# Blaizzy/mlx-audio

Hardware: AMD Instinct MI355X
Metric: audio samples/sec + real-time factor, Kokoro-82M TTS (higher is better)
Workload: dtype bf16 weights x fp32 activations: vocoder convs = fp16 hi pass (v_mfma_f32_32x32x16_f16) + block-scaled FP4 (e2m1) lo pass (v_mfma_scale_f32_32x32x64_f8f6f4 cbsz / blgp 4, OCP MX: E8M0 scale per row x 32 channels / per output column), fp32 accumulate; front end bf16 hi+lo split; 1 GPU; Kokoro-82M bf16 TTS, tokens->waveform, canonical short sentence T=80 F=264 (6.6 s @ 24 kHz); utterances_per_gpu=64, global_batch=64, samples_per_utterance=158400, parallelism=utterance-dp1, precision_mode=6, wire=fp32

## Files before the change

include/mi355audio.h:

```cpp
#ifndef MI355AUDIO_H
#define MI355AUDIO_H

#include <stdint.h>

#ifdef __cplusplus
extern "C" {
#endif

#define MI355_OK 0
#define MI355_ERR_ARG (-1)
#define MI355_ERR_LAUNCH (-2)
#define MI355_ERR_UNSUPPORTED (-3)

const char* mi355_last_error(void);
int mi355_abi_version(void);
int mi355_device_info(int dev, char* name, int name_cap, int* cu_count, int* lds_bytes);

enum { MI355_ACT_NONE = 0, MI355_ACT_LEAKY = 1, MI355_ACT_SNAKE = 2, MI355_ACT_GELU = 3,
       MI355_ACT_ELU = 4,
       MI355_ACT_SILU = 5,
       MI355_ACT_GELU_TANH = 6,
       MI355_ACT_TANH = 7 };

typedef struct {
// ... 334 lines not shown
  float* y; int64_t y_rstride;
} mi355_interp1d_args;
int mi355_interpolate1d(const mi355_interp1d_args* a, void* stream);

int mi355_conv1d_c1_k3s2(const float* x, int32_t ldx_b, int32_t Lin, const int32_t* lens_in,
                         float w0, float w1, float w2, float bias, float* y, int64_t y_bstride, int32_t ldy, int32_t col,
                         int32_t Lout, int32_t B, void* stream);

typedef struct {
  const float* f0; int32_t ld_f0; int32_t L2; const int32_t* lens2; int32_t B;
  int32_t up; int32_t H; float sr; float sine_amp; float noise_std; float voiced_thr;
  const float* rand_ini; const float* noise;
  const float* lin_w; float lin_b;
  float* phase_ws;
  float* out; int32_t ld_out;
  float* quant_ws;
  int32_t coarse_f32;
} mi355_sine_source_args;
int mi355_sine_source(const mi355_sine_source_args* a, void* stream);

typedef struct {
  const float* x; int32_t ldx; int32_t L; const int32_t* lens; int32_t B;
  int32_t n_fft; int32_t hop; const float* window;
  float* y; int64_t y_bstride; int32_t ldy;
} mi355_stft_magphase_args;
int mi355_stft_magphase(const mi355_stft_magphase_args* a, void* stream);

typedef struct {
  const float* x; int64_t x_bstride; int32_t ldx; int32_t Fr; const int32_t* lens; int32_t B;
  int32_t n_fft; int32_t hop; const float* window;
  float* audio; int32_t ld_audio;
} mi355_istft_head_args;
int mi355_istft_head(const mi355_istft_head_args* a, void* stream);

typedef struct {
  const float* x; int64_t x_bstride; int32_t ldx; int32_t Cin; int32_t L; const int32_t* lens; int32_t B;
  const uint16_t* w; const float* bias; int32_t Cout; int32_t K; int32_t dil; int32_t pad;
  int32_t pre_act; float pre_slope; int32_t precision;
  int32_t n_fft; int32_t hop; const float* window;
  float* audio; int32_t ld_audio;
} mi355_conv_post_istft_args;
int mi355_conv_post_istft(const mi355_conv_post_istft_args* a, void* stream);

typedef struct {
  const float* x; int64_t x_bstride; int32_t ldx; int32_t Cin; int32_t L; const int32_t* lens; int32_t B;
  const uint16_t* w; const float* bias; int32_t Cout; int32_t K; int32_t u; int32_t p; int32_t row_off;
  float slope; int32_t precision;
  const float* res; int64_t res_bstride; int32_t ldr;
  float* y; int64_t y_bstride; int32_t ldy;
} mi355_upsample_polyphase_args;
int mi355_upsample_polyphase(const mi355_upsample_polyphase_args* a, void* stream);

typedef struct {
  const float* x; int32_t ldx; int32_t L; int32_t B;
  int32_t n_fft; int32_t hop; const float* window;
  int32_t pad_mode; int32_t n_frames;
  float* out;
} mi355_stft_args;
int mi355_stft(const mi355_stft_args* a, void* stream);

typedef struct {
  const float* x; int32_t ldx; int32_t L; int32_t B;
  int32_t n_fft; int32_t hop; const float* window; int32_t pad_mode; int32_t n_frames;
  const float* fb; int32_t n_mels; int32_t mode;
  float* out;
  float* gmax;
  float log_guard;
} mi355_logmel_args;
int mi355_logmel(const mi355_logmel_args* a, void* stream);
int mi355_logmel_finish(float* y, int64_t n_per_item, const float* gmax, int32_t B, void* stream);

typedef struct {
  const float* x; int32_t L;
  int32_t win; int32_t shift; int32_t pad; int32_t n_fft; int32_t n_frames;
  const float* window;
  const float* noise;
  float dither; float preemph;
  float* frames;
} mi355_kaldi_frames_args;
int mi355_kaldi_frames(const mi355_kaldi_frames_args* a, void* stream);
int mi355_polar_spec(const float* x, int64_t x_bstride, int32_t ldx, int32_t Fr, int32_t nb, int32_t B, float clip, float* spec, void* stream);


typedef struct {
  const float* spec; int32_t n_frames; int32_t B;
  int32_t n_fft; int32_t hop; const float* window; const float* norm;
  int32_t norm_mode;
  int32_t clamp; int32_t trim; int32_t out_len;
  float* frames_ws;
  float* out; int32_t ld_out;
} mi355_istft_args;
int mi355_istft(const mi355_istft_args* a, void* stream);

enum { MI355_KV_F32 = 0, MI355_KV_BF16 = 1, MI355_KV_F16 = 2 };
typedef struct {
  const float* q; int64_t q_bstride; int32_t ldq;
  const float* k; int64_t k_bstride; int32_t ldk;
  const float* v; int64_t v_bstride; int32_t ldv;
  int32_t heads; int32_t kv_heads; int32_t dh;
  int32_t Tq; int32_t Tk;
  const int32_t* lens_q;
  const int32_t* lens_k;
  int32_t causal; int32_t window; float scale;
  int32_t B;
  int32_t mode;
  float* out; int64_t out_bstride; int32_t ldo;
// ... 443 lines not shown
```

mlx_audio_amd/build.py:

```python
from __future__ import annotations

import hashlib
import os
import shutil
import subprocess
import sys

HERE = os.path.dirname(os.path.abspath(__file__))
CSRC = os.path.join(HERE, "csrc")
LIBDIR = os.path.join(HERE, "lib")
LIBPATH = os.path.join(LIBDIR, "libmi355audio.so")
HEADER = os.path.join(os.path.dirname(HERE), "include", "mi355audio.h")
SOURCES = ["api.cpp", "conv_gemm.hip", "conv_ws4.hip", "conv_ws4_p4.hip", "conv_ws4_p13.hip", "conv_ws4_p5.hip", "conv_ws4_p6.hip", "conv_ws4_p5_probe.hip", "conv_ws4_fq.hip", "upsample_poly.hip", "conv_quant.hip", "norm.hip", "group_norm.hip", "s3.hip", "conformer.hip", "narrow_attn.hip", "mid_attn.hip", "align.hip", "lstm.hip", "lstm_seq.hip", "gru.hip", "dfn.hip", "bandsplit.hip", "sanm.hip", "mossformer.hip", "attention.hip", "glue.hip", "source.hip", "fft.hip", "flash_attn.hip",
           "decode_rules.hip", "gemv.hip", "gemv_mfma.hip", "gemv_mfma_fp8.hip", "gemm_rows.hip", "rows_pipe.hip", "transformer.hip", "rvq.hip", "ecapa.hip", "sampler.hip", "stack_step.cpp", "firered.hip"]
EXTRA_FLAGS = {"source.hip": ["-ffp-contract=off"], "dfn.hip": ["-ffp-contract=off"]}
COMMON_FLAGS = ["-fno-slp-vectorize"]


def _hipcc() -> str:
    for cand in (os.environ.get("HIPCC"), shutil.which("hipcc"), "/opt/rocm/bin/hipcc"):
        if cand and os.path.exists(cand):
            return cand
    raise RuntimeError("hipcc not found (set HIPCC=/path/to/hipcc)")


def _fingerprint() -> str:
    h = hashlib.sha256()
    for name in SOURCES + sorted(n for n in os.listdir(CSRC) if n.endswith(".h")):
        with open(os.path.join(CSRC, name), "rb") as f:
            h.update(f.read())
    with open(HEADER, "rb") as f:
        h.update(f.read())
    h.update(repr(sorted(EXTRA_FLAGS.items())).encode())
    h.update(repr(COMMON_FLAGS).encode())
    return h.hexdigest()


def build(force: bool = False, verbose: bool = True) -> str:
    os.makedirs(LIBDIR, exist_ok=True)
    stamp = os.path.join(LIBDIR, "libmi355audio.stamp")
    fp = _fingerprint()
    if not force and os.path.exists(LIBPATH) and os.path.exists(stamp) and open(stamp).read().strip() == fp:
        return LIBPATH
    hipcc = _hipcc()
    objs = []
    objdir = os.path.join(LIBDIR, "obj")
    os.makedirs(objdir, exist_ok=True)
    procs = []
    for src in SOURCES:
        obj = os.path.join(objdir, src.rsplit(".", 1)[0] + ".o")
        objs.append(obj)
        cmd = [hipcc, "--offload-arch=gfx950", "-O3", "-std=c++17", "-fPIC", *COMMON_FLAGS, *EXTRA_FLAGS.get(src, []), "-x", "hip", "-c",
               os.path.join(CSRC, src), "-o", obj]
        if verbose:
            print("[build]", " ".join(cmd), flush=True)
        procs.append((src, subprocess.Popen(cmd, stdout=subprocess.PIPE, stderr=subprocess.STDOUT, text=True)))
    for src, p in procs:
        out, _ = p.communicate()
        if p.returncode != 0:
            raise RuntimeError(f"hipcc failed on {src}:\n{out}")
        if verbose and out.strip():
            print(out)
    link = [hipcc, "--offload-arch=gfx950", "-shared", "-fPIC", "-o", LIBPATH] + objs
    if verbose:
        print("[build]", " ".join(link), flush=True)
    r = subprocess.run(link, stdout=subprocess.PIPE, stderr=subprocess.STDOUT, text=True)
# ... 10 lines not shown
```

mlx_audio_amd/ops.py:

```python
from __future__ import annotations

import ctypes
import math
import os
from dataclasses import dataclass
from typing import Optional, Tuple

import numpy as np
import torch

from . import _lib

ACT_NONE, ACT_LEAKY, ACT_SNAKE, ACT_GELU, ACT_ELU, ACT_SILU, ACT_GELU_TANH, ACT_TANH = 0, 1, 2, 3, 4, 5, 6, 7

PROFILE = None


def _stream() -> int:
    return torch.cuda.current_stream().cuda_stream


def profile_finalize(entries):
    torch.cuda.synchronize()
    out = []
# ... 1557 lines not shown
            PROFILE.append(((L * B) if lens is None else lens.sum(), pc.cin, pc.cout, pc.k, dil, 0, e0, e1))
        _lib.call_struct("mi355_conv_post_istft", "mi355_conv_post_istft_args", _stream(), x=_ptr(x), x_bstride=xbs, ldx=ldx, Cin=pc.cin, L=L,
                         lens=_ptr(lens), B=B, w=_ptr(pc.w), bias=_ptr(pc.bias), Cout=pc.cout, K=pc.k, dil=dil, pad=pad, pre_act=pre_act,
                         pre_slope=pre_slope, precision=precision, n_fft=n_fft, hop=hop, window=_ptr(window), audio=_ptr(audio),
                         ld_audio=audio.stride(0))
        if PROFILE is not None:
            e1.record()
        return audio
    post = torch.empty((B, L, round_up(pc.cout, 4)), dtype=torch.float32, device=x.device)[:, :, :pc.cout]
    conv_gemm(x, pc, post, dil=dil, pad=pad, lens_in=lens, lens_out=lens, pre_act=pre_act, pre_slope=pre_slope, precision=precision, pre_fq=pre_fq)
    return istft_head(post, n_fft, hop, window, audio, lens=lens)


UPSAMPLE_POLY_SHAPES = {(512, 256, 10): 32, (256, 128, 6): 64}


def upsample_polyphase_eligible(pc: PackedConv, stride: int, *, pre_act: int = ACT_LEAKY, precision: int = 2, res=True, pre_fq=None) -> bool:
    return (pc.k == 2 and stride > 0 and pc.cout % stride == 0 and (pc.cin, pc.cout // stride, stride) in UPSAMPLE_POLY_SHAPES
            and pre_act == ACT_LEAKY and precision == 2 and not pc.f16 and not pc.mx and res is not None and pre_fq is None)


def upsample_polyphase(x: torch.Tensor, pc: PackedConv, res: torch.Tensor, y: torch.Tensor, stride: int, *, row_off: int = 0, lens=None,
                       pre_act: int = ACT_LEAKY, pre_slope: float = 0.1, precision: int = 2, pre_fq=None):
    B, L, _, xbs, ldx = _nlc(x)
    u = stride
    cout = pc.cout // u
    kfull = pc.k * u
    p = (kfull - u) // 2
    Lo = L * u + row_off
    assert y.shape[0] == B and y.shape[1] >= Lo and y.shape[2] == cout and res.shape[0] == B and res.shape[1] >= Lo and res.shape[2] == cout
    if upsample_polyphase_eligible(pc, u, pre_act=pre_act, precision=precision, res=res, pre_fq=pre_fq) and row_off in (0, 1):
        _, _, _, rbs, ldr = _nlc(res)
        _, _, _, ybs, ldy = _nlc(y)
        assert pc.w.numel() >= _lib.load().mi355_packed_conv_weight_elems(pc.cout, pc.k, pc.cin)
        if PROFILE is not None:
            e0, e1 = torch.cuda.Event(enable_timing=True), torch.cuda.Event(enable_timing=True)
            e0.record()
            PROFILE.append((((L + 1) * B) if lens is None else (lens + 1).sum(), pc.cin, pc.cout, pc.k, 1, 1, e0, e1))
        _lib.call_struct("mi355_upsample_polyphase", "mi355_upsample_polyphase_args", _stream(), x=_ptr(x), x_bstride=xbs, ldx=ldx, Cin=pc.cin, L=L,
                         lens=_ptr(lens), B=B, w=_ptr(pc.w), bias=_ptr(pc.bias), Cout=cout, K=kfull, u=u, p=p, row_off=row_off, slope=pre_slope,
                         precision=precision, res=_ptr(res), res_bstride=rbs, ldr=ldr, y=_ptr(y), y_bstride=ybs, ldy=ldy)
        if PROFILE is not None:
            e1.record()
        return y
    kp = pc.k
    conv_gemm(x, pc, y, pad=kp - 1, lout=L + kp - 1, lens_in=lens, lens_out=None if lens is None else lens + (kp - 1), pre_act=pre_act,
              pre_slope=pre_slope, res=res, precision=precision, pre_fq=pre_fq,
              up=dict(s=u, p=p, cout=cout, row_off=row_off, lout=L * u, lens=None if lens is None else lens * u))
    if row_off:
        y[:, :row_off, :].copy_(res[:, :row_off, :])
    return y


def stft_frames(x: torch.Tensor, n_fft: int, hop: int, window: torch.Tensor, pad_mode: int, n_frames: int):
    assert x.dim() == 2 and x.stride(1) == 1 and x.dtype == torch.float32
    B, L = x.shape
    out = torch.empty((B, n_frames, n_fft // 2 + 1, 2), dtype=torch.float32, device=x.device)
    _lib.call_struct("mi355_stft", "mi355_stft_args", _stream(), x=_ptr(x), ldx=x.stride(0), L=L, B=B, n_fft=n_fft, hop=hop,
                     window=_ptr(window), pad_mode=pad_mode, n_frames=n_frames, out=_ptr(out))
    return torch.view_as_complex(out)


def logmel(x: torch.Tensor, n_fft: int, hop: int, window: torch.Tensor, pad_mode: int, n_frames: int, fb: torch.Tensor,
           mode: int, log_guard: float = 0.0, fixed_max: Optional[float] = None):
    assert x.dim() == 2 and x.stride(1) == 1 and fb.is_contiguous()
    B, L = x.shape
    n_mels = fb.shape[0]
    out = torch.empty((B, n_frames, n_mels), dtype=torch.float32, device=x.device)
    gmax = torch.empty((B,), dtype=torch.float32, device=x.device) if mode == 0 else None
    _lib.call_struct("mi355_logmel", "mi355_logmel_args", _stream(), x=_ptr(x), ldx=x.stride(0), L=L, B=B, n_fft=n_fft,
                     hop=hop, window=_ptr(window), pad_mode=pad_mode, n_frames=n_frames, fb=_ptr(fb), n_mels=n_mels,
                     mode=mode, out=_ptr(out), gmax=None if fixed_max is not None else _ptr(gmax), log_guard=float(log_guard))
    if mode == 0:
        if fixed_max is not None:
            gmax.fill_(float(fixed_max))
        lib = _lib.load()
        rc = lib.mi355_logmel_finish(_ptr(out), n_frames * n_mels, _ptr(gmax), B, _stream())
        _lib.check(rc, "mi355_logmel_finish")
    return out


def kaldi_frames(x: torch.Tensor, win: int, shift: int, pad: int, n_fft: int, n_frames: int, window: torch.Tensor, preemph: float,
                 noise: Optional[torch.Tensor] = None, dither: float = 0.0) -> torch.Tensor:
    assert x.dim() == 1 and x.is_contiguous() and x.dtype == torch.float32 and window.numel() == win
    out = torch.empty((n_frames, n_fft), dtype=torch.float32, device=x.device)
    if noise is not None:
        assert noise.is_contiguous() and tuple(noise.shape) == (n_frames, win)
    _lib.call_struct("mi355_kaldi_frames", "mi355_kaldi_frames_args", _stream(), x=_ptr(x), L=x.numel(), win=win, shift=shift, pad=pad, n_fft=n_fft,
                     n_frames=n_frames, window=_ptr(window), noise=_ptr(noise), dither=dither, preemph=preemph, frames=_ptr(out))
    return out


def polar_spec(x: torch.Tensor, nb: int, clip: float = 1e2) -> torch.Tensor:
    B, Fr, C, xbs, ldx = _nlc(x)
    assert C >= 2 * nb
    spec = torch.empty((B, Fr, nb), dtype=torch.complex64, device=x.device)
    lib = _lib.load()
    rc = lib.mi355_polar_spec(_ptr(x), xbs, ldx, Fr, nb, B, float(clip), _ptr(torch.view_as_real(spec)), _stream())
    _lib.check(rc, "mi355_polar_spec")
    return spec


def istft_frames(spec: torch.Tensor, n_fft: int, hop: int, window: torch.Tensor, norm: torch.Tensor, norm_mode: int,
                 clamp: bool, trim: int, out_len: int):
    sr = torch.view_as_real(spec.contiguous())
    B, n_frames = spec.shape[0], spec.shape[1]
# ... 121 lines not shown
```

mlx_audio_amd/tts/models/kokoro/engine.py:

```python
from __future__ import annotations

import math
import os
from dataclasses import dataclass, field
from typing import Dict, List, Optional, Sequence

import numpy as np
import torch

from .... import ops
from ....ops import ACT_GELU, ACT_GELU_TANH, ACT_LEAKY, ACT_NONE, ACT_SNAKE, PackedConv, round_up


def fold_weight_norm(v: torch.Tensor, g: torch.Tensor, param_dtype: torch.dtype) -> torch.Tensor:
    v_ = v.to(param_dtype)
    g_ = g.to(param_dtype)
    axes = tuple(range(1, v_.dim()))
    nrm = torch.sqrt((v_ * v_).sum(dim=axes, keepdim=True))
    w = (v_ / (nrm + torch.tensor(1e-7, dtype=param_dtype))) * g_
    return w.to(torch.float32)


@dataclass
class _AdaIN:
# ... 92 lines not shown
        return torch.cat([hdr, self.ids[i].to(torch.int32).view(torch.float32), self.dur[i].to(torch.int32).view(torch.float32),
                          self.ref_s[i].reshape(-1).to(torch.float32), self.d[i].reshape(-1).to(torch.float32)])

    @staticmethod
    def packed_size(T: int, style: int, width: int) -> int:
        return 1 + 2 * T + style + T * width

    @classmethod
    def unpack(cls, blobs: Sequence[torch.Tensor], frames: Sequence[int], style: int, width: int, speed: float = 1.0) -> "KokoroFront":
        ids, dur, ref, d = [], [], [], []
        for b in blobs:
            T = (int(b.numel()) - 1 - style) // (2 + width)
            ids.append(b[1:1 + T].view(torch.int32))
            dur.append(b[1 + T:1 + 2 * T].view(torch.int32))
            ref.append(b[1 + 2 * T:1 + 2 * T + style])
            d.append(b[1 + 2 * T + style:].reshape(T, width))
        return cls(ids, torch.stack(ref, 0), d, dur, list(frames), speed, None)

    @classmethod
    def concat(cls, parts: Sequence["KokoroFront"]) -> "KokoroFront":
        parts = [p for p in parts if len(p.ids)]
        return cls(sum((p.ids for p in parts), []), torch.cat([p.ref_s for p in parts], 0), sum((p.d for p in parts), []),
                   sum((p.dur for p in parts), []), sum((list(p.frames) for p in parts), []), parts[0].speed, None)


class KokoroEngine:
    ffn_act = ACT_GELU
    alpha_name = "alpha{w}.{i}"
    max_frames = 0
    coarse_f32 = False

    def _decoder_dims(self, config: dict):
        return 1024, 512, 64

    @staticmethod
    def default_precision(param_dtype, quant_modules: Sequence[str] = ()) -> int:
        if param_dtype == torch.float32:
            return 4
        return 6 if (param_dtype == torch.bfloat16 and not tuple(quant_modules)) else 2

    def __init__(self, weights: Dict[str, torch.Tensor], config: dict, device="cuda", param_dtype=torch.bfloat16,
                 precision: Optional[int] = None, quant_modules: Sequence[str] = ()):
        ops.require_gpu()
        self.cfg = config
        self.qmods = tuple(quant_modules)
        if precision is None:
            precision = self.default_precision(param_dtype, self.qmods)
        self.all_f16 = precision == 4
        self.cdim, self.gdim, self.adim = self._decoder_dims(config)
        self.dev = torch.device(device)
        self.pdt = param_dtype
        self.precision = precision
        self.fuse_stats = True
        self.fold_quant = os.environ.get("MI355_FOLD_QUANT", "1") != "0"
        self.ext_partials = os.environ.get("MI355_EXT_PARTIALS", "1") != "0"
        self.w = weights
        ist = config["istftnet"]
        self.rates = [int(r) for r in ist["upsample_rates"]]
        self.kers = [int(k) for k in ist["upsample_kernel_sizes"]]
        self.n_fft, self.hop = int(ist["gen_istft_n_fft"]), int(ist["gen_istft_hop_size"])
        self.total_up = int(np.prod(self.rates)) * self.hop
        self.rk = list(ist["resblock_kernel_sizes"])
        self.rd = [list(d) for d in ist["resblock_dilation_sizes"]]
        self.hid = config["hidden_dim"]
        self.sty = config["style_dim"]
        self.n_layer = config["n_layer"]
        self.pb = config["plbert"]
        self.bank_dec = _StyleBank()
        self.bank_pred = _StyleBank()
        self._load()

    def _t(self, name) -> torch.Tensor:
        return self.w[name].to(torch.float32)

    def _q(self, t: torch.Tensor) -> torch.Tensor:
        return t.to(self.pdt).to(torch.float32)

    def _lin(self, pre, bias=True) -> PackedConv:
        return ops.pack_conv(self._q(self._t(f"{pre}.weight")), self._q(self._t(f"{pre}.bias")) if bias else None, self.dev, f16=self.all_f16)

    def _wn(self, pre) -> torch.Tensor:
        return fold_weight_norm(self.w[f"{pre}.weight_v"], self.w[f"{pre}.weight_g"], self.pdt)

    def _convw(self, pre, bias=True) -> PackedConv:
        b = self._q(self._t(f"{pre}.bias")) if bias and f"{pre}.bias" in self.w else None
        w = self._wn(pre)
        mx = (self.precision in (5, 6) and pre.startswith("decoder.") and w.dim() == 3 and ops.mx_pays(w.shape[0], w.shape[1], w.shape[2])
              and not (self.qmods and self._isq(pre)))
        return ops.pack_conv(w, b, self.dev, f16=self._f16(pre), mx=(2 if self.precision == 6 else 1) if mx else 0)

    def _f16(self, pre: str) -> bool:
        return self.all_f16 or (self.precision == 3 and pre.startswith("decoder."))

    def _dvec(self, t: torch.Tensor, pad_to: int = 0) -> torch.Tensor:
        t = self._q(t.reshape(-1).float())
        if pad_to and t.numel() < pad_to:
            t = torch.cat([t, torch.ones(pad_to - t.numel())])
        return t.contiguous().to(self.dev)

    def _isq(self, name: str) -> bool:
        return any(q == name or q.startswith(name + ".") for q in self.qmods)

    def _adain(self, bank: _StyleBank, pre, c) -> _AdaIN:
        q = self._isq(pre)
        bank.any_q = bank.any_q or q
        return _AdaIN(bank.add(self._q(self._t(f"{pre}.fc.weight")), self._q(self._t(f"{pre}.fc.bias"))), c, q)
# ... 27 lines not shown
                          [self._adain(bank, f"{pre}.adain2.{i}", ch) for i in range(3)],
                          [self._dvec(self._t(f"{pre}.{self.alpha_name.format(w=1, i=i)}"), cp) for i in range(3)],
                          [self._dvec(self._t(f"{pre}.{self.alpha_name.format(w=2, i=i)}"), cp) for i in range(3)], k, dils, ch, pre)

    def _load(self):
        d, hid, sty = self.dev, self.hid, self.sty
        e = "bert.embeddings"
        self.word_emb = self._q(self._t(f"{e}.word_embeddings.weight")).contiguous().to(d)
        self.pos_emb = self._q(self._t(f"{e}.position_embeddings.weight")).contiguous().to(d)
        self.type_row = self._q(self._t(f"{e}.token_type_embeddings.weight"))[0].contiguous().to(d)
        self.emb_ln = (self._dvec(self._t(f"{e}.LayerNorm.weight")), self._dvec(self._t(f"{e}.LayerNorm.bias")))
        self.map_in = self._lin("bert.encoder.embedding_hidden_mapping_in")
        lay = "bert.encoder.albert_layer_groups.0.albert_layers.0"
        qkv_w = torch.cat([self._q(self._t(f"{lay}.attention.{n}.weight")) for n in ("query", "key", "value")], 0)
        qkv_b = torch.cat([self._q(self._t(f"{lay}.attention.{n}.bias")) for n in ("query", "key", "value")], 0)
        self.qkv = ops.pack_conv(qkv_w, qkv_b, d, f16=self.all_f16)
        self.att_dense = self._lin(f"{lay}.attention.dense")
        self.att_ln = (self._dvec(self._t(f"{lay}.attention.LayerNorm.weight")), self._dvec(self._t(f"{lay}.attention.LayerNorm.bias")))
        self.ffn = self._lin(f"{lay}.ffn")
        self.ffn_out = self._lin(f"{lay}.ffn_output")
        self.full_ln = (self._dvec(self._t(f"{lay}.full_layer_layer_norm.weight")), self._dvec(self._t(f"{lay}.full_layer_layer_norm.bias")))
        self.bert_encoder = self._lin("bert_encoder")
        self.dur_lstms = [self._lstm(f"predictor.text_encoder.lstms.{2 * i}") for i in range(self.n_layer)]
        self.dur_adaln = [self._adain(self.bank_pred, f"predictor.text_encoder.lstms.{2 * i + 1}", hid) for i in range(self.n_layer)]
        self.pred_lstm = self._lstm("predictor.lstm")
        self.dur_proj = self._lin("predictor.duration_proj.linear_layer")
        self.shared = self._lstm("predictor.shared")
        self.f0_blocks, self.n_blocks = [], []
        dims = [(hid, hid), (hid, hid // 2), (hid // 2, hid // 2)]
        for i, (a, b) in enumerate(dims):
            self.f0_blocks.append(self._resblk1d(self.bank_pred, f"predictor.F0.{i}", a, b))
            self.n_blocks.append(self._resblk1d(self.bank_pred, f"predictor.N.{i}", a, b))
        self.f0_proj = ops.pack_conv(self._q(self._t("predictor.F0_proj.weight")), self._q(self._t("predictor.F0_proj.bias")), d, f16=self.all_f16)
        self.n_proj = ops.pack_conv(self._q(self._t("predictor.N_proj.weight")), self._q(self._t("predictor.N_proj.bias")), d, f16=self.all_f16)
        self.te_emb = self._q(self._t("text_encoder.embedding.weight")).contiguous().to(d)
        self.te_cnn = []
        for i in range(self.n_layer):
            self.te_cnn.append((self._convw(f"text_encoder.cnn.{i}.0"), self._dvec(self._t(f"text_encoder.cnn.{i}.1.weight")),
                                self._dvec(self._t(f"text_encoder.cnn.{i}.1.bias"))))
        self.te_k = self.w["text_encoder.cnn.0.0.weight_v"].shape[1]
        self.te_lstm = self._lstm("text_encoder.lstm")
        cd, gd, ad = self.cdim, self.gdim, self.adim
        self.enc_blk = self._resblk1d(self.bank_dec, "decoder.encode", hid + 2, cd)
        self.dec_blks = [self._resblk1d(self.bank_dec, f"decoder.decode.{i}", cd + 2 + ad, cd if i < 3 else gd) for i in range(4)]
        f0w, nw = self._wn("decoder.F0_conv").reshape(-1), self._wn("decoder.N_conv").reshape(-1)
        self.f0_conv = ([float(v) for v in f0w], float(self._q(self._t("decoder.F0_conv.bias"))[0]))
        self.n_conv = ([float(v) for v in nw], float(self._q(self._t("decoder.N_conv.bias"))[0]))
        self.asr_res = self._convw("decoder.asr_res.0")
        g = "decoder.generator"
        self.src_w = self._dvec(self._t(f"{g}.m_source.l_linear.weight"))
        self.src_b = float(self._q(self._t(f"{g}.m_source.l_linear.bias"))[0])
        c0 = int(self.cfg["istftnet"]["upsample_initial_channel"])
        nk = len(self.rk)
        self.ups, self.noise_convs, self.noise_res, self.resblocks = [], [], [], []
        for i, (u, k) in enumerate(zip(self.rates, self.kers)):
            cout = c0 // (2 ** (i + 1))
            w_t = self._wn(f"{g}.ups.{i}").permute(2, 1, 0).contiguous()
            self.ups.append(ops.pack_conv_transpose(w_t, self._q(self._t(f"{g}.ups.{i}.bias")), u, d, f16=self.precision == 3 or self.all_f16))
            ncw = self._q(self._t(f"{g}.noise_convs.{i}.weight"))
            ncb = self._q(self._t(f"{g}.noise_convs.{i}.bias"))
            nbp = ops.round_up(ncw.shape[2], 4)
            ncwp = torch.zeros((ncw.shape[0], ncw.shape[1], nbp), dtype=ncw.dtype)
            ncwp[:, :, : ncw.shape[2]] = ncw
            self.noise_convs.append(ops.pack_conv(ncwp.reshape(ncw.shape[0], 1, -1) if ncw.shape[1] > 1 else ncw, ncb, d, f16=self.all_f16))
            last = i + 1 == len(self.rates)
            self.noise_res.append(self._resblock1(self.bank_dec, f"{g}.noise_res.{i}", cout, 11 if last else 7, (1, 3, 5)))
            for j in range(nk):
                self.resblocks.append(self._resblock1(self.bank_dec, f"{g}.resblocks.{i * nk + j}", cout, self.rk[j], tuple(self.rd[j])))
        self.conv_post = self._convw(f"{g}.conv_post")
        self.style_dec = self.bank_dec.pack(d, self.all_f16)
        self.style_pred = self.bank_pred.pack(d, self.all_f16)
        self.q_style_dec, self.q_style_pred = self.bank_dec.any_q, self.bank_pred.any_q
        n = self.n_fft
        self.window = torch.tensor([0.5 * (1 - math.cos(2 * math.pi * i / n)) for i in range(n)], dtype=torch.float32, device=d)
        self.w = None

    def _new(self, *shape, zero=False):
        return (torch.zeros if zero else torch.empty)(shape, dtype=torch.float32, device=self.dev)

    def _gb(self, gb_all: _StyleProj, a: _AdaIN) -> torch.Tensor:
        return (gb_all.quant if a.q else gb_all.plain)[:, a.off: a.off + 2 * a.c]

    def _style_proj(self, s: torch.Tensor, pc: PackedConv, quant: bool) -> _StyleProj:
        B = s.shape[0]
        plain = self._new(1, B, pc.cout)
        self._conv(s[None, :, :], pc, plain)
        q = None
        if quant:
            q = self._new(1, B, pc.cout)
            sq = ops.fake_quant_u8(s[:, None, :])
            self._conv(sq.as_strided((1, B, sq.shape[2]), (B * sq.stride(0), sq.stride(0), 1)), pc, q)
            q = q[0]
        return _StyleProj(plain[0], q)

    def _prec(self, pc) -> int:
        return 2 if (self.precision == 3 or (self.precision in (5, 6) and not pc.f16)) else self.precision

    def _conv(self, x, pc, y, **kw):
        kw.setdefault("precision", self._prec(pc))
        return ops.conv_gemm(x, pc, y, **kw)

    def _convq(self, name: str, x, pc, y, *, lens_in=None, pre=None, pre_act=ACT_NONE, pre_slope=0.0, pre_alpha=None, ext_in=None, ext_out=None, ret_ext=False, **kw):
        want = ret_ext
        done = None
        if self.qmods and self._isq(name):
            if self.fold_quant and "flat" not in kw:
                if ext_in is not None:
                    mm = ops.fake_quant_extrema_from_partials(ext_in, x.shape[1], lens=lens_in, pre=pre, pre_act=pre_act, pre_slope=pre_slope, pre_alpha=pre_alpha)
                else:
                    mm = ops.fake_quant_extrema(x, lens=lens_in, pre=pre, pre_act=pre_act, pre_slope=pre_slope, pre_alpha=pre_alpha)
                if ext_out is not None and self.ext_partials and ops.conv_ext_supported(x, pc, B=x.shape[0], lout=kw.get("lout") or y.shape[1], dil=kw.get("dil", 1), pre_act=pre_act,
                                                                         post_act=kw.get("post_act", ACT_NONE), up=kw.get("up"), precision=self._prec(pc)):
                    kw["ext"] = done = ext_out
                self._conv(x, pc, y, lens_in=lens_in, pre=pre, pre_act=pre_act, pre_slope=pre_slope, pre_alpha=pre_alpha, pre_fq=mm, **kw)
# ... 267 lines not shown
            assert tuple(n_curve.shape) == (B, 2 * Fm)

        f0_in, n_in = f0_curve, n_curve
        if self.qmods and self._isq("decoder.F0_conv"):
            f0_in = ops.fake_quant_u8(f0_curve[:, :, None], y=torch.zeros_like(f0_curve)[:, :, None], lens=lens_2f)[:, :, 0]
        if self.qmods and self._isq("decoder.N_conv"):
            n_in = ops.fake_quant_u8(n_curve[:, :, None], y=torch.zeros_like(n_curve)[:, :, None], lens=lens_2f)[:, :, 0]
        ops.conv1d_c1_k3s2(f0_in, self.f0_conv[0], self.f0_conv[1], dec_in, hid, lens_in=lens_2f)
        ops.conv1d_c1_k3s2(n_in, self.n_conv[0], self.n_conv[1], dec_in, hid + 1, lens_in=lens_2f)
        cd, gd, ad = self.cdim, self.gdim, self.adim
        c_cat = cd + ad + 2
        ca = self._new(B, Fm, round_up(c_cat, 32), zero=True)
        cb = self._new(B, Fm, round_up(c_cat, 32), zero=True)
        trace = {}
        self._resblk1d_fwd(self.enc_blk, dec_in[:, :, :c_in], gb_dec, ca[:, :, :cd], lens_f)
        if return_intermediates:
            trace.update(dec_in=dec_in[:, :, :c_in].clone(), enc=ca[:, :, :cd].clone())
        self._convq("decoder.asr_res.0", asr, self.asr_res, ca[:, :, cd:cd + ad], lens_in=lens_f, lens_out=lens_f, flatten=True)
        ca[:, :, cd + ad:c_cat].copy_(dec_in[:, :, hid:hid + 2])
        cb[:, :, cd:c_cat].copy_(ca[:, :, cd:c_cat])
        cur, nxt = ca, cb
        for i in range(3):
            self._resblk1d_fwd(self.dec_blks[i], cur[:, :, :c_cat], gb_dec, nxt[:, :, :cd], lens_f)
            cur, nxt = nxt, cur
            if return_intermediates:
                trace[f"dec{i}"] = cur[:, :, :cd].clone()
        xg = self._new(B, 2 * Fm, gd)
        self._resblk1d_fwd(self.dec_blks[3], cur[:, :, :c_cat], gb_dec, xg, lens_f, lens_2f)

        up = self.total_up
        L2 = 2 * Fm
        if rand_ini is None or noise is None:
            gen = torch.Generator(device=dev).manual_seed(noise_seed)
            rand_ini = torch.rand((B, 9), generator=gen, device=dev, dtype=torch.float32)
            noise = torch.randn((B, L2 * up, 9), generator=gen, device=dev, dtype=torch.float32)
        rand_ini = rand_ini.to(dev).contiguous()
        noise = noise.to(dev).contiguous()
        g_n = "decoder.generator"
        har_src = ops.sine_source(f0_curve, rand_ini, noise, self.src_w, self.src_b, up, lens2=lens_2f,
                                  quant=bool(self.qmods) and self._isq(f"{g_n}.m_source.l_linear"), coarse_f32=self.coarse_f32)
        nb2 = self.n_fft + 2
        nbp = ops.round_up(nb2, 4)
        n_har = L2 * up // self.hop + 1
        har = self._new(B, n_har, nbp, zero=True)[:, :, :nb2]
        lens_samples = frames * (2 * up) if ragged else None
        ops.stft_magphase(har_src, self.n_fft, self.hop, self.window, har, lens=lens_samples)
        if "har" in overrides:
            har.copy_(overrides["har"].to(device=dev, dtype=torch.float32))
        lens_har = lens_samples // self.hop + 1 if ragged else None
        x = xg
        L = L2
        lens_x = lens_2f
        nk = len(self.rk)
        for i, (u, k) in enumerate(zip(self.rates, self.kers)):
            last = i + 1 == len(self.rates)
            cout = self.ups[i].cout // u
            Lo = L * u + (1 if last else 0)
            lens_o = (lens_x * u + (1 if last else 0)) if ragged else None
            xsrc = self._new(B, Lo, cout)
            har_i = har
            if self.qmods and self._isq(f"{g_n}.noise_convs.{i}"):
                har_i = ops.fake_quant_u8(har, y=self._new(B, n_har, nbp, zero=True)[:, :, :nb2], lens=lens_har)
            if not last:
                sf = int(np.prod(self.rates[i + 1:]))
                self._conv(har_i, self.noise_convs[i], xsrc, lens_in=lens_har, lens_out=lens_o,
                           flat=dict(ldx=sf * nbp, x_off=-((sf + 1) // 2) * nbp, channels=nbp))
            else:
                self._conv(har_i, self.noise_convs[i], xsrc, lens_in=lens_har, lens_out=lens_o)
            if return_intermediates:
                trace[f"nconv{i}"] = xsrc.clone()
            xsrc = self._resblock1_fwd(self.noise_res[i], xsrc, gb_dec, lens_o)
            if return_intermediates:
                trace[f"nres{i}"] = xsrc.clone()
            kp = k // u
            xu = self._new(B, Lo, cout)
            lens_gemm = (lens_x + (kp - 1)) if ragged else None
            lens_ct = (lens_x * u) if ragged else None
            if not (self.qmods and self._isq(f"{g_n}.ups.{i}")) and ops.upsample_polyphase_eligible(self.ups[i], u, precision=self._prec(self.ups[i])):
                ops.upsample_polyphase(x, self.ups[i], xsrc, xu, u, row_off=1 if last else 0, lens=lens_x, pre_slope=0.1, precision=self._prec(self.ups[i]))
            else:
                self._convq(f"{g_n}.ups.{i}", x, self.ups[i], xu, pad=kp - 1, lout=L + kp - 1, lens_in=lens_x, lens_out=lens_gemm, pre_act=ACT_LEAKY,
                            pre_slope=0.1, res=xsrc, up=dict(s=u, p=(k - u) // 2, cout=cout, row_off=1 if last else 0, lout=L * u, lens=lens_ct))
                if last:
                    xu[:, 0, :].copy_(xsrc[:, 0, :])
            if return_intermediates:
                trace[f"xu{i}"] = xu.clone()
            acc = self._new(B, Lo, cout)
            xu_sums = torch.empty(B * cout * 2, dtype=torch.float64, device=dev)
            for j in range(nk):
                self._resblock1_fwd(self.resblocks[i * nk + j], xu, gb_dec, lens_o, out=acc, accumulate=j > 0,
                                    out_scale=(1.0 / nk) if j == nk - 1 else 1.0, x_sums=(xu_sums, j > 0))
            x, L, lens_x = acc, Lo, lens_o
            if return_intermediates:
                trace[f"stage{i}"] = acc.clone()
        audio = self._new(B, (L - 1) * self.hop, zero=True)
        post = None
        if not return_intermediates and not (self.qmods and self._isq(f"{g_n}.conv_post")):
            ops.conv_post_istft(x, self.conv_post, self.n_fft, self.hop, self.window, audio, lens=lens_x, pre_slope=0.01, precision=self._prec(self.conv_post))
        else:
            post = self._new(B, L, round_up(nb2, 4))
            self._convq(f"{g_n}.conv_post", x, self.conv_post, post[:, :, :nb2], pad=3, lens_in=lens_x, lens_out=lens_x, pre_act=ACT_LEAKY, pre_slope=0.01)
            ops.istft_head(post[:, :, :nb2], self.n_fft, self.hop, self.window, audio, lens=lens_x)
        outs = [audio[b, : Fs[b] * 2 * up] for b in range(B)]
        durs = [dur[b, : Ts[b]] for b in range(B)]
        if return_intermediates:
            return outs, durs, dict(d=d, en=en, f0=f0_curve, n=n_curve, asr=asr, t_en=t_en, dur_raw=dur_raw, har_src=har_src,
                                    har=har, bert=h, xg=xg, post=post[:, :, :nb2], dec3=xg, **trace)
        return outs, durs
```

Baseline: 202.2 million samples/s.

## Fuse both harmonic noise convs into one kernel with fused stats epilogue

Adds a dedicated HIP kernel that loads the harmonic STFT tile once into LDS as a bf16 hi/lo split and computes both noise_convs stages (the strided 12-tap conv and the 1x1 conv) from it, writing outputs plus per-block statistics partials. The engine uses it when shapes match and passes the precomputed stats to the second resblock. This replaces two separate conv launches and a second read of the har tensor, and saves a stats pass. It is specialised to one fixed shape and precision, and the first stage's stats are computed but not consumed.

```diff
diff --git a/include/mi355audio.h b/include/mi355audio.h
--- a/include/mi355audio.h
+++ b/include/mi355audio.h
@@ -410,6 +410,16 @@
 int mi355_upsample_polyphase(const mi355_upsample_polyphase_args* a, void* stream);
 
 typedef struct {
+  const float* har; int64_t har_bstride; int32_t ld_har; int32_t C; int32_t n_har; const int32_t* lens0; int32_t L0; int32_t B;
+  const uint16_t* w0; const float* bias0; int32_t Cout0; int32_t K0; int32_t stride0;
+  const uint16_t* w1; const float* bias1; int32_t Cout1; int32_t K1;
+  int32_t precision;
+  float* y0; int64_t y0_bstride; int32_t ldy0; float* stats0; int64_t stats0_bstride;
+  float* y1; int64_t y1_bstride; int32_t ldy1; float* stats1; int64_t stats1_bstride;
+} mi355_har_noise_convs_args;
+int mi355_har_noise_convs(const mi355_har_noise_convs_args* a, void* stream);
+
+typedef struct {
   const float* x; int32_t ldx; int32_t L; int32_t B;
   int32_t n_fft; int32_t hop; const float* window;
   int32_t pad_mode; int32_t n_frames;
diff --git a/mlx_audio_amd/build.py b/mlx_audio_amd/build.py
--- a/mlx_audio_amd/build.py
+++ b/mlx_audio_amd/build.py
@@ -11,7 +11,7 @@
 LIBDIR = os.path.join(HERE, "lib")
 LIBPATH = os.path.join(LIBDIR, "libmi355audio.so")
 HEADER = os.path.join(os.path.dirname(HERE), "include", "mi355audio.h")
-SOURCES = ["api.cpp", "conv_gemm.hip", "conv_ws4.hip", "conv_ws4_p4.hip", "conv_ws4_p13.hip", "conv_ws4_p5.hip", "conv_ws4_p6.hip", "conv_ws4_p5_probe.hip", "conv_ws4_fq.hip", "upsample_poly.hip", "conv_quant.hip", "norm.hip", "group_norm.hip", "s3.hip", "conformer.hip", "narrow_attn.hip", "mid_attn.hip", "align.hip", "lstm.hip", "lstm_seq.hip", "gru.hip", "dfn.hip", "bandsplit.hip", "sanm.hip", "mossformer.hip", "attention.hip", "glue.hip", "source.hip", "fft.hip", "flash_attn.hip",
+SOURCES = ["api.cpp", "conv_gemm.hip", "conv_ws4.hip", "conv_ws4_p4.hip", "conv_ws4_p13.hip", "conv_ws4_p5.hip", "conv_ws4_p6.hip", "conv_ws4_p5_probe.hip", "conv_ws4_fq.hip", "upsample_poly.hip", "har_convs.hip", "conv_quant.hip", "norm.hip", "group_norm.hip", "s3.hip", "conformer.hip", "narrow_attn.hip", "mid_attn.hip", "align.hip", "lstm.hip", "lstm_seq.hip", "gru.hip", "dfn.hip", "bandsplit.hip", "sanm.hip", "mossformer.hip", "attention.hip", "glue.hip", "source.hip", "fft.hip", "flash_attn.hip",
            "decode_rules.hip", "gemv.hip", "gemv_mfma.hip", "gemv_mfma_fp8.hip", "gemm_rows.hip", "rows_pipe.hip", "transformer.hip", "rvq.hip", "ecapa.hip", "sampler.hip", "stack_step.cpp", "firered.hip"]
 EXTRA_FLAGS = {"source.hip": ["-ffp-contract=off"], "dfn.hip": ["-ffp-contract=off"]}
 COMMON_FLAGS = ["-fno-slp-vectorize"]
diff --git a/mlx_audio_amd/csrc/har_convs.hip b/mlx_audio_amd/csrc/har_convs.hip
--- /dev/null
+++ b/mlx_audio_amd/csrc/har_convs.hip
@@ -0,0 +1,209 @@
+#include "conv_common.h"
+
+using namespace mi355conv;
+
+namespace {
+
+constexpr int kHarThreads = 512;
+constexpr int kLd = 24;
+constexpr int kTile0 = 128, kTile1 = 768;
+constexpr int kLead = 3;
+constexpr int kWinRows = kTile1 + 6;
+constexpr int kPlane = kWinRows * kLd * 2;
+constexpr int kC0 = 256, kC1 = 128, kChunks0 = 9;
+
+struct har_args {
+  const float* har; int64_t har_bstride; int n_har; const int32_t* lens0; int L0;
+  mi355_conv_gemm_args e0, e1;
+  const char* w0; const char* w1;
+};
+
+__global__ __launch_bounds__(kHarThreads, 4) void har_noise_convs_kernel(const har_args a, const int ntiles) {
+  extern __shared__ __attribute__((aligned(16))) char smem[];
+  char* const A_hi = smem;
+  char* const A_lo = smem + kPlane;
+
+  const int tid = threadIdx.x, lane = tid & 63;
+  const int wave = __builtin_amdgcn_readfirstlane(tid >> 6);
+  const int hl = lane & 31, hh = lane >> 5;
+  const int b = (int)blockIdx.x / ntiles;
+  const int t = (int)blockIdx.x - b * ntiles;
+  const int raw = a.lens0 ? a.lens0[b] : a.L0;
+  const int len0 = raw < 0 ? 0 : (raw > a.L0 ? a.L0 : raw);
+  const int len1 = 6 * len0 + 1;
+  if (t * kTile1 >= len1) return;
+
+  const int wm = wave >> 2, wn = wave & 3;
+  const bool act0 = t * kTile0 + wm * 64 < len0;
+  const char* const wf0 = a.w0 + (wn * 4) * 1024 + lane * 16;
+  bf16x8 bw[2][4];
+  auto load_w0 = [&](const int chunk) {
+#pragma unroll
+    for (int f = 0; f < 4; ++f) bw[chunk & 1][f] = *(const bf16x8*)(wf0 + chunk * 16384 + f * 1024);
+  };
+  if (act0) load_w0(0);
+
+  {
+    constexpr int TOTAL = kWinRows * kLd / 4;
+    constexpr int NIT = (TOTAL + kHarThreads - 1) / kHarThreads;
+    const float* const xb = a.har + (int64_t)b * a.har_bstride;
+    const int e0 = (t * kTile1 - kLead) * (kLd / 4);
+    const int evalid = len1 * (kLd / 4), emax = a.n_har * (kLd / 4) - 1;
+    float4 v[NIT];
+#pragma unroll
+    for (int i = 0; i < NIT; ++i) {
+      int e = e0 + tid + i * kHarThreads;
+      e = e < 0 ? 0 : (e > emax ? emax : e);
+      v[i] = *(const float4*)(xb + (int64_t)e * 4);
+    }
+#pragma unroll
+    for (int i = 0; i < NIT; ++i) {
+      const int idx = tid + i * kHarThreads;
+      if (idx < TOTAL) {
+        const int e = e0 + idx;
+        const bool ok = e >= 0 && e < evalid;
+        const float in[4] = {v[i].x, v[i].y, v[i].z, v[i].w};
+        float tt[4];
+#pragma unroll
+        for (int j = 0; j < 4; ++j) {
+          const float u = in[j] + 0.0f;
+          tt[j] = ok ? u : 0.f;
+        }
+        uint2 ph, pl;
+        ph.x = pack_bf16x2(tt[0], tt[1]);
+        ph.y = pack_bf16x2(tt[2], tt[3]);
+        const float h0 = __builtin_bit_cast(float, ph.x << 16), h1 = __builtin_bit_cast(float, ph.x & 0xffff0000u);
+        const float h2 = __builtin_bit_cast(float, ph.y << 16), h3 = __builtin_bit_cast(float, ph.y & 0xffff0000u);
+        pl.x = pack_bf16x2(tt[0] - h0, tt[1] - h1);
+        pl.y = pack_bf16x2(tt[2] - h2, tt[3] - h3);
+        *(uint2*)(A_hi + idx * 8) = ph;
+        *(uint2*)(A_lo + idx * 8) = pl;
+      }
+    }
+  }
+  __syncthreads();
+
+  if (act0) {
+    f32x16 acc[2][2];
+#pragma unroll
+    for (int mf = 0; mf < 2; ++mf)
+#pragma unroll
+      for (int nf = 0; nf < 2; ++nf)
+#pragma unroll
+        for (int r = 0; r < 16; ++r) acc[mf][nf][r] = 0.f;
+    const int arow = (wm * 64 + hl) * (6 * kLd * 2) + hh * 16;
+#pragma unroll
+    for (int chunk = 0; chunk < kChunks0; ++chunk) {
+      if (chunk + 1 < kChunks0) load_w0(chunk + 1);
+      asm volatile("" ::: "memory");
+#pragma unroll
+      for (int kk = 0; kk < 2; ++kk) {
+        bf16x8 ah[2], al[2];
+#pragma unroll
+        for (int mf = 0; mf < 2; ++mf) {
+          const int addr = arow + mf * (32 * 6 * kLd * 2) + (chunk * 2 + kk) * 32;
+          ah[mf] = *(const bf16x8*)(A_hi + addr);
+          al[mf] = *(const bf16x8*)(A_lo + addr);
+        }
+#pragma unroll
+        for (int mf = 0; mf < 2; ++mf) {
+#pragma unroll
+          for (int nf = 0; nf < 2; ++nf) acc[mf][nf] = mfma16<2>(ah[mf], bw[chunk & 1][nf * 2 + kk], acc[mf][nf]);
+#pragma unroll
+          for (int nf = 0; nf < 2; ++nf) acc[mf][nf] = mfma16<2>(al[mf], bw[chunk & 1][nf * 2 + kk], acc[mf][nf]);
+        }
+      }
+    }
+    const int row0 = t * kTile0 + wm * 64;
+    if (row0 + 64 <= len0) conv_epilogue_interior<2, 2, 64, 64>(a.e0, acc, b, row0, wn * 64, 0, 0, lane);
+    else conv_epilogue<2, 2, 64, 64, 0>(a.e0, acc, b, row0, wn * 64, 0, 0, lane, len0, false);
+  }
+
+  {
+    const int wn1 = wave & 1;
+    for (int blk = wave >> 1; blk < kTile1 / 64; blk += 4) {
+      const int row0 = t * kTile1 + blk * 64;
+      if (row0 >= len1) break;
+      int ln = lane;
+      asm volatile("" : "+v"(ln));
+      const int bl = ln & 31, bh = ln >> 5;
+      const char* const wf1 = a.w1 + (wn1 * 4) * 1024 + ln * 16;
+      bf16x8 b1[4];
+#pragma unroll
+      for (int f = 0; f < 4; ++f) b1[f] = *(const bf16x8*)(wf1 + f * 1024);
+      f32x16 acc[2][2];
+#pragma unroll
+      for (int mf = 0; mf < 2; ++mf)
+#pragma unroll
+        for (int nf = 0; nf < 2; ++nf)
+#pragma unroll
+          for (int r = 0; r < 16; ++r) acc[mf][nf][r] = 0.f;
+#pragma unroll
+      for (int kk = 0; kk < 2; ++kk) {
+        const bool pad = kk == 1 && bh == 1;
+        bf16x8 ah[2], al[2];
+#pragma unroll
+        for (int mf = 0; mf < 2; ++mf) {
+          const int addr = (blk * 64 + mf * 32 + bl + kLead) * (kLd * 2) + kk * 32 + (pad ? 0 : bh * 16);
+          ah[mf] = *(const bf16x8*)(A_hi + addr);
+          al[mf] = *(const bf16x8*)(A_lo + addr);
+          if (pad) {
+#pragma unroll
+            for (int j = 0; j < 8; ++j) { ah[mf][j] = 0; al[mf][j] = 0; }
+          }
+        }
+#pragma unroll
+        for (int mf = 0; mf < 2; ++mf) {
+#pragma unroll
+          for (int nf = 0; nf < 2; ++nf) acc[mf][nf] = mfma16<2>(ah[mf], b1[nf * 2 + kk], acc[mf][nf]);
+#pragma unroll
+          for (int nf = 0; nf < 2; ++nf) acc[mf][nf] = mfma16<2>(al[mf], b1[nf * 2 + kk], acc[mf][nf]);
+        }
+      }
+      if (row0 + 64 <= len1) conv_epilogue_interior<2, 2, 64, 64>(a.e1, acc, b, row0, wn1 * 64, 0, 0, ln);
+      else conv_epilogue<2, 2, 64, 64, 0>(a.e1, acc, b, row0, wn1 * 64, 0, 0, ln, len1, false);
+    }
+  }
+}
+
+}
+
+extern "C" int mi355_har_noise_convs(const mi355_har_noise_convs_args* ap, void* stream) {
+  MI355_REQUIRE(ap && ap->har && ap->w0 && ap->w1 && ap->y0 && ap->y1 && ap->stats0 && ap->stats1, "har_noise_convs: null tensor");
+  const mi355_har_noise_convs_args p = *ap;
+  if (p.C != 22 || p.ld_har != kLd || p.Cout0 != kC0 || p.K0 != 12 || p.stride0 != 6 || p.Cout1 != kC1 || p.K1 != 1 || p.precision != 2) {
+    mi355_set_error("har_noise_convs: unsupported shape (C=%d ld_har=%d stage 0: Cout=%d K=%d stride=%d, stage 1: Cout=%d K=%d, precision=%d)", p.C,
+                    p.ld_har, p.Cout0, p.K0, p.stride0, p.Cout1, p.K1, p.precision);
+    return MI355_ERR_UNSUPPORTED;
+  }
+  const int64_t L1 = (int64_t)p.L0 * 6 + 1;
+  MI355_REQUIRE(p.B > 0 && p.L0 >= 0 && p.n_har >= L1 && p.ldy0 >= kC0 && p.ldy1 >= kC1, "har_noise_convs: bad shape");
+  MI355_REQUIRE(p.B == 1 || (p.har_bstride >= (int64_t)p.n_har * kLd && p.y0_bstride >= (int64_t)p.L0 * p.ldy0 && p.y1_bstride >= L1 * p.ldy1),
+                "har_noise_convs: items overlap");
+  MI355_REQUIRE(L1 * p.ldy1 < ((int64_t)1 << 29) && (int64_t)p.n_har * kLd < ((int64_t)1 << 29), "har_noise_convs: an item's rows exceed the 32-bit byte offsets");
+  MI355_REQUIRE((p.har_bstride & 3) == 0 && (((uintptr_t)p.har | (uintptr_t)p.w0 | (uintptr_t)p.w1) & 15) == 0, "har_noise_convs: har rows must be 16-byte aligned");
+  MI355_REQUIRE(p.stats0_bstride >= ((int64_t)p.L0 + 63) / 64 * kC0 * 2 && p.stats1_bstride >= (L1 + 63) / 64 * kC1 * 2, "har_noise_convs: statistics buffers too small");
+  MI355_REQUIRE((((uintptr_t)p.stats0 | (uintptr_t)p.stats1) & 7) == 0 && (p.stats0_bstride & 1) == 0 && (p.stats1_bstride & 1) == 0, "har_noise_convs: statistics must be 8-byte aligned");
+
+  har_args a{};
+  a.har = p.har; a.har_bstride = p.har_bstride; a.n_har = p.n_har; a.lens0 = p.lens0; a.L0 = p.L0;
+  a.w0 = (const char*)p.w0; a.w1 = (const char*)p.w1;
+  a.e0.y = p.y0; a.e0.y_bstride = p.y0_bstride; a.e0.ldy = p.ldy0; a.e0.bias = p.bias0; a.e0.Cout = kC0; a.e0.out_scale = 1.0f;
+  a.e0.stats_partial = p.stats0; a.e0.stats_bstride = p.stats0_bstride;
+  a.e1.y = p.y1; a.e1.y_bstride = p.y1_bstride; a.e1.ldy = p.ldy1; a.e1.bias = p.bias1; a.e1.Cout = kC1; a.e1.out_scale = 1.0f;
+  a.e1.stats_partial = p.stats1; a.e1.stats_bstride = p.stats1_bstride;
+
+  constexpr int lds = 2 * kPlane;
+  static bool attr_set = false;
+  if (!attr_set) {
+    hipError_t e = hipFuncSetAttribute((const void*)har_noise_convs_kernel, hipFuncAttributeMaxDynamicSharedMemorySize, lds);
+    MI355_REQUIRE(e == hipSuccess, "har_noise_convs: cannot reserve %d bytes of LDS: %s", lds, hipGetErrorString(e));
+    attr_set = true;
+  }
+  const int ntiles = p.L0 / kTile0 + 1;
+  MI355_REQUIRE((int64_t)p.B * ntiles < (int64_t)1 << 31, "har_noise_convs: too many tiles");
+  MI355_CLEAR_ERROR();
+  hipLaunchKernelGGL(har_noise_convs_kernel, dim3((unsigned)(p.B * ntiles)), dim3(kHarThreads), lds, (hipStream_t)stream, a, ntiles);
+  MI355_LAUNCH_CHECK("har_noise_convs");
+  return MI355_OK;
+}
diff --git a/mlx_audio_amd/ops.py b/mlx_audio_amd/ops.py
--- a/mlx_audio_amd/ops.py
+++ b/mlx_audio_amd/ops.py
@@ -1633,6 +1633,37 @@
     return y
 
 
+def har_noise_convs_eligible(pc0: PackedConv, pc1: PackedConv, n_bins: int, taps0: int, stride0: int, *, precision: int = 2, pre_fq=None) -> bool:
+    return (n_bins == 22 and taps0 == 12 and stride0 == 6 and pc0.k == 1 and pc0.cin == taps0 * round_up(n_bins, 4) and pc0.cout == 256
+            and pc1.k == 1 and pc1.cin == n_bins and pc1.cout == 128 and precision == 2 and not (pc0.f16 or pc0.mx or pc1.f16 or pc1.mx) and pre_fq is None)
+
+
+def har_noise_convs(har: torch.Tensor, pc0: PackedConv, pc1: PackedConv, xsrc0: torch.Tensor, xsrc1: torch.Tensor, stats0: torch.Tensor,
+                    stats1: torch.Tensor, lens0: Optional[torch.Tensor] = None, *, taps0: int = 12, stride0: int = 6, precision: int = 2):
+    B, n_har, C, hbs, ldh = _nlc(har)
+    B0, L0, C0, y0bs, ldy0 = _nlc(xsrc0)
+    B1, L1, C1, y1bs, ldy1 = _nlc(xsrc1)
+    if not har_noise_convs_eligible(pc0, pc1, C, taps0, stride0, precision=precision):
+        raise _lib.Mi355Error("har_noise_convs: not a shape of mi355_har_noise_convs (see har_noise_convs_eligible)")
+    assert B0 == B and B1 == B and C0 == pc0.cout and C1 == pc1.cout and L1 >= stride0 * L0 + 1 and n_har >= stride0 * L0 + 1
+    for st, L, c in ((stats0, L0, C0), (stats1, stride0 * L0 + 1, C1)):
+        assert st.dtype == torch.float32 and st.dim() == 4 and st.is_contiguous() and st.shape[0] == B and st.shape[2] == c and st.shape[3] == 2
+        assert st.shape[1] >= (L + STATS_ROWS - 1) // STATS_ROWS
+    if PROFILE is not None:
+        e0, e1 = torch.cuda.Event(enable_timing=True), torch.cuda.Event(enable_timing=True)
+        e0.record()
+        PROFILE.append(((L0 * B) if lens0 is None else lens0.sum(), pc0.cin, pc0.cout, pc0.k, 1, 0, e0, e1))
+        PROFILE.append((((stride0 * L0 + 1) * B) if lens0 is None else (lens0 * stride0 + 1).sum(), pc1.cin, pc1.cout, pc1.k, 1, 0, e1, e1))
+    _lib.call_struct("mi355_har_noise_convs", "mi355_har_noise_convs_args", _stream(), har=_ptr(har), har_bstride=hbs, ld_har=ldh, C=C, n_har=n_har,
+                     lens0=_ptr(lens0), L0=L0, B=B, w0=_ptr(pc0.w), bias0=_ptr(pc0.bias), Cout0=pc0.cout, K0=taps0, stride0=stride0,
+                     w1=_ptr(pc1.w), bias1=_ptr(pc1.bias), Cout1=pc1.cout, K1=pc1.k, precision=precision,
+                     y0=_ptr(xsrc0), y0_bstride=y0bs, ldy0=ldy0, stats0=_ptr(stats0), stats0_bstride=stats0.stride(0),
+                     y1=_ptr(xsrc1), y1_bstride=y1bs, ldy1=ldy1, stats1=_ptr(stats1), stats1_bstride=stats1.stride(0))
+    if PROFILE is not None:
+        e1.record()
+    return xsrc0, xsrc1
+
+
 def stft_frames(x: torch.Tensor, n_fft: int, hop: int, window: torch.Tensor, pad_mode: int, n_frames: int):
     assert x.dim() == 2 and x.stride(1) == 1 and x.dtype == torch.float32
     B, L = x.shape
diff --git a/mlx_audio_amd/tts/models/kokoro/engine.py b/mlx_audio_amd/tts/models/kokoro/engine.py
--- a/mlx_audio_amd/tts/models/kokoro/engine.py
+++ b/mlx_audio_amd/tts/models/kokoro/engine.py
@@ -168,6 +168,8 @@
         self.pdt = param_dtype
         self.precision = precision
         self.fuse_stats = True
+        self.fuse_har = True
+        self.fuse_har_stats = (False, True)
         self.fold_quant = os.environ.get("MI355_FOLD_QUANT", "1") != "0"
         self.ext_partials = os.environ.get("MI355_EXT_PARTIALS", "1") != "0"
         self.w = weights
@@ -301,7 +303,7 @@
         self.src_b = float(self._q(self._t(f"{g}.m_source.l_linear.bias"))[0])
         c0 = int(self.cfg["istftnet"]["upsample_initial_channel"])
         nk = len(self.rk)
-        self.ups, self.noise_convs, self.noise_res, self.resblocks = [], [], [], []
+        self.ups, self.noise_convs, self.noise_taps, self.noise_res, self.resblocks = [], [], [], [], []
         for i, (u, k) in enumerate(zip(self.rates, self.kers)):
             cout = c0 // (2 ** (i + 1))
             w_t = self._wn(f"{g}.ups.{i}").permute(2, 1, 0).contiguous()
@@ -309,6 +311,7 @@
             ncw = self._q(self._t(f"{g}.noise_convs.{i}.weight"))
             ncb = self._q(self._t(f"{g}.noise_convs.{i}.bias"))
             nbp = ops.round_up(ncw.shape[2], 4)
+            self.noise_taps.append(int(ncw.shape[1]))
             ncwp = torch.zeros((ncw.shape[0], ncw.shape[1], nbp), dtype=ncw.dtype)
             ncwp[:, :, : ncw.shape[2]] = ncw
             self.noise_convs.append(ops.pack_conv(ncwp.reshape(ncw.shape[0], 1, -1) if ncw.shape[1] > 1 else ncw, ncb, d, f16=self.all_f16))
@@ -682,16 +685,32 @@
         L = L2
         lens_x = lens_2f
         nk = len(self.rk)
+        har_fused = None
+        if (self.fuse_har and self.fuse_stats and len(self.rates) == 2 and not (self.qmods and any(self._isq(f"{g_n}.noise_convs.{i}") for i in range(2)))
+                and ops.har_noise_convs_eligible(self.noise_convs[0], self.noise_convs[1], nb2, self.noise_taps[0], self.rates[1],
+                                                 precision=max(self._prec(self.noise_convs[0]), self._prec(self.noise_convs[1])))):
+            L0, L1 = L2 * self.rates[0], L2 * self.rates[0] * self.rates[1] + 1
+            xs0, xs1 = self._new(B, L0, self.noise_convs[0].cout), self._new(B, L1, self.noise_convs[1].cout)
+            st0, st1 = ops.new_stats(B, L0, xs0.shape[2], dev), ops.new_stats(B, L1, xs1.shape[2], dev)
+            ops.har_noise_convs(har, self.noise_convs[0], self.noise_convs[1], xs0, xs1, st0, st1, (lens_2f * self.rates[0]) if ragged else None,
+                                taps0=self.noise_taps[0], stride0=self.rates[1])
+            har_fused = [(xs0, st0), (xs1, st1)]
+            del xs0, xs1, st0, st1
         for i, (u, k) in enumerate(zip(self.rates, self.kers)):
             last = i + 1 == len(self.rates)
             cout = self.ups[i].cout // u
             Lo = L * u + (1 if last else 0)
             lens_o = (lens_x * u + (1 if last else 0)) if ragged else None
-            xsrc = self._new(B, Lo, cout)
+            if har_fused is not None:
+                (xsrc, xsrc_stats), har_fused[i] = har_fused[i], None
+            else:
+                xsrc, xsrc_stats = self._new(B, Lo, cout), None
             har_i = har
             if self.qmods and self._isq(f"{g_n}.noise_convs.{i}"):
                 har_i = ops.fake_quant_u8(har, y=self._new(B, n_har, nbp, zero=True)[:, :, :nb2], lens=lens_har)
-            if not last:
+            if har_fused is not None:
+                pass
+            elif not last:
                 sf = int(np.prod(self.rates[i + 1:]))
                 self._conv(har_i, self.noise_convs[i], xsrc, lens_in=lens_har, lens_out=lens_o,
                            flat=dict(ldx=sf * nbp, x_off=-((sf + 1) // 2) * nbp, channels=nbp))
@@ -699,7 +718,7 @@
                 self._conv(har_i, self.noise_convs[i], xsrc, lens_in=lens_har, lens_out=lens_o)
             if return_intermediates:
                 trace[f"nconv{i}"] = xsrc.clone()
-            xsrc = self._resblock1_fwd(self.noise_res[i], xsrc, gb_dec, lens_o)
+            xsrc = self._resblock1_fwd(self.noise_res[i], xsrc, gb_dec, lens_o, x_stats=xsrc_stats if self.fuse_har_stats[i] else None)
             if return_intermediates:
                 trace[f"nres{i}"] = xsrc.clone()
             kp = k // u
```

Result: no change. 204.2 million samples/s, median of 6 (+1.0%).
